# LoganWilliams1/mhm2_kmer_analysis_v2

Hardware: AMD Instinct MI355X
Metric: k-mers/sec (kcount stage) at k=21 (higher is better)
Workload: dtype u64

## Files before the change

### mhm2_kmer_analysis_v2_amd/csrc/kc_api.hip

```cpp
#include <hip/hip_runtime.h>

#include <math.h>
#include <stdio.h>
#include <stdlib.h>
#include <string.h>

#include <algorithm>
#include <new>
#include <thread>
#include <string>
#include <type_traits>
#include <unordered_map>
#include <vector>

#include "../../include/kcount_mi355.h"
#include "kc_bucketed.hpp"
#include "kc_shard.hpp"
#include "kc_wire6.hpp"
#include "kc_supermer.hpp"
#include "kc_ctg.hpp"
#include "kc_merge.hpp"
#include "kc_trim.hpp"
#include "kc_fastq.hpp"

// ... 30 lines not shown
                                               "kc_trim_sizes_kernel", "kc_merge_scan_kernel<trim>", "kc_trim_write_kernel"};
struct kt_pending {
  hipEvent_t start, stop;
  int kind;
};

struct kc_ctx {
  kc_config cfg;
  std::vector<kt_pending> kt_pend;
  uint64_t kt_launches[KT_COUNT];
  double kt_ms[KT_COUNT];
  int k, nl;
  int nl_ext;
  hipStream_t own_stream, stream;
  uint8_t *arena;
  size_t arena_bytes;
  uint64_t capacity;
  Table table;
  uint64_t *d_ctrs;
  uint64_t *h_ctrs;
  uint64_t *d_tile_first;
  uint64_t *d_out_plan;
  size_t tile_first_cap;
  uint8_t *d_stage_bases, *d_stage_quals;
  uint64_t *d_stage_offsets;
  size_t stage_bytes, stage_reads;
  struct {
    uint8_t *d_bases[2], *d_quals[2], *h_bases[2], *h_quals[2];
    uint64_t *d_offs[2], *h_offs[2];
    hipEvent_t copied[2], consumed[2], half[2];
    uint32_t lead_b[2], lead_q[2];
    bool used[2];
    hipStream_t copy_stream, copy_stream2;
    size_t cap_bytes, cap_reads;
    bool ready;
  } hp;
  uint64_t *d_out_keys;
  uint64_t *d_out_keys_ext;
  uint16_t *d_out_counts;
  uint8_t *d_out_left, *d_out_right;
  uint64_t out_cap, out_n;
  bool finalized;
  uint32_t *d_index;
  uint64_t index_cap;
  Table ctg_table;
  uint64_t ctg_cap;
// ... 376 lines not shown
  if (c->d_out_keys_ext) (void)hipFree(c->d_out_keys_ext);
  c->d_out_keys_ext = nullptr;
  if (c->d_out_counts) (void)hipFree(c->d_out_counts);
  if (c->d_out_left) (void)hipFree(c->d_out_left);
  if (c->d_out_right) (void)hipFree(c->d_out_right);
  c->d_out_keys = nullptr;
  c->d_out_counts = nullptr;
  c->d_out_left = c->d_out_right = nullptr;
  c->out_cap = c->out_n = 0;
}

extern "C" void kc_destroy(kc_ctx *c) {
  if (!c) return;
  (void)hipSetDevice(c->cfg.device);
  if (c->stream) (void)hipStreamSynchronize(c->stream);
  drain_kernel_times(c);
  free_results(c);
  if (c->arena) (void)hipFree(c->arena);
  if (c->d_ctrs) (void)hipFree(c->d_ctrs);
  if (c->d_w6cur) (void)hipFree(c->d_w6cur);
  if (c->d_l2snap) (void)hipFree(c->d_l2snap);
  if (c->h_ctrs) (void)hipHostFree(c->h_ctrs);
  if (c->d_tile_first) (void)hipFree(c->d_tile_first);
  if (c->d_out_plan) (void)hipFree(c->d_out_plan);
  if (c->d_stage_bases) (void)hipFree(c->d_stage_bases);
  if (c->d_stage_quals) (void)hipFree(c->d_stage_quals);
  if (c->d_stage_offsets) (void)hipFree(c->d_stage_offsets);
  if (c->d_synth) (void)hipFree(c->d_synth);
  if (c->d_sm_bytes) (void)hipFree(c->d_sm_bytes);
  if (c->d_sm_packed) (void)hipFree(c->d_sm_packed);
  if (c->d_sm_targets) (void)hipFree(c->d_sm_targets);
  if (c->d_sm_out) (void)hipFree(c->d_sm_out);
  if (c->d_sm_ctr) (void)hipFree(c->d_sm_ctr);
  if (c->d_mg) (void)hipFree(c->d_mg);
  if (c->d_ad) (void)hipFree(c->d_ad);
  if (c->d_tr) (void)hipFree(c->d_tr);
  if (c->d_fq_text) (void)hipFree(c->d_fq_text);
  if (c->d_fq_tiles) (void)hipFree(c->d_fq_tiles);
  if (c->d_fq_recs) (void)hipFree(c->d_fq_recs);
  host_pipe_free(c);
  free_ctg(c);
  bk_free(c, false);
  shard_free(c);
  if (c->d_cb) (void)hipFree(c->d_cb);
  if (c->h_cb) (void)hipHostFree(c->h_cb);
  if (c->own_stream) (void)hipStreamDestroy(c->own_stream);
// ... 307 lines not shown
    if (!rc) rc = bk_take(c, 10, (void **)&b.ovf2, b.ovf2_cap * w);
    if (!rc) rc = bk_take(c, 11, (void **)&b.done1, nseg * 4);
    if (!rc) rc = bk_take(c, 12, (void **)&b.used2, (size_t)g.P1 * 4);
    if (rc) return rc;
  }
  if (getenv("KC_DEBUG_ADDR"))
    fprintf(stderr, "kc arenas: rec1 %p (%zu MB) chain1 %p cnt1 %p rec2 %p chain2 %p ovf1 %p ovf2 %p\n", (void *)b.rec1, rec1_bytes >> 20,
            (void *)b.chain1, (void *)b.cnt1, (void *)b.rec2, (void *)b.chain2, (void *)b.ovf1, (void *)b.ovf2);
  c->bk_bytes = rec1_bytes + rec2_bytes + (b.ovf1_cap + b.ovf2_cap) * w + nseg * (g.L1MAX + 1) * 4 + (size_t)R * (g.L2MAX + 2) * 4;
  c->bk_capacity = bcap;
  c->bk_ready = true;
  c->bk_rot = 0;
  int rc = bk_empty_level1(c);
  if (!rc) rc = bk_empty_level2(c);
  return rc;
}

static int sync_cb(kc_ctx *c) {
  HIPCHK(hipMemcpyAsync(c->h_cb, c->d_cb, CB_COUNT * 8, hipMemcpyDeviceToHost, c->stream));
  HIPCHK(hipStreamSynchronize(c->stream));
  return KC_OK;
}

static int bk_ovf1_room(kc_ctx *c, uint64_t want, uint64_t *room) {
  if (c->ovf1_ub + want <= c->bb.ovf1_cap) {
    *room = c->bb.ovf1_cap - c->ovf1_ub;
    return KC_OK;
  }
  int rc = sync_cb(c);
  if (rc) return rc;
  if (c->h_cb[CB_FATAL] & ~(c->inc_on ? (uint64_t)FATAL_OVF2 : 0ULL)) {
    snprintf(g_last_error, sizeof(g_last_error), "k-mer buffer: records were lost (fatal bits %llu)", (unsigned long long)c->h_cb[CB_FATAL]);
    return KC_ERR_CAPACITY;
  }
  uint64_t used = std::min<uint64_t>(c->h_cb[CB_OVF1], c->bb.ovf1_cap);
  if (used && c->bb.ovf1_cap - used < want && !c->sh.extracting) {
    rc = ensure_room(c, used);
    if (rc) return rc;
    {
      KernelTimer kt(c, KT_FALLBACK);
      with_nl(c, [&](auto nl) {
        auto kern = with_cp<nl>(c, [&](auto cp) { return kc_ovf1_drain_kernel<nl, cp>; });
        hipLaunchKernelGGL(kern, dim3((unsigned)std::min<uint64_t>((used + TPB - 1) / TPB, 256 * 32)), dim3(TPB), 0, c->stream, c->gm, c->bb,
                           used, c->table, c->d_ctrs);
      });
    }
    HIPCHK(hipGetLastError());
    HIPCHK(hipMemsetAsync(c->d_cb + CB_OVF1, 0, 8, c->stream));
    used = 0;
  }
  c->ovf1_ub = used;
  *room = c->bb.ovf1_cap - used;
  return KC_OK;
}

template <typename K>
static int set_dyn_lds(K kernel, size_t bytes) {
  HIPCHK(hipFuncSetAttribute((const void *)kernel, hipFuncAttributeMaxDynamicSharedMemorySize, (int)bytes));
  return KC_OK;
}

template <int NL> static size_t lds_l1_reads() {
  return ((sizeof(L1LDS) + 15) & ~size_t(15)) + Rnd<NL>::STAGE_READS + ((size_t)WGB * Rnd<NL>::RPOS_READS + 64) * 2;
}
template <int NL> static size_t lds_bin_reads() { return (sizeof(L1LDS) + 15) & ~size_t(15); }
template <int NL> static size_t lds_l1_records() { return ((sizeof(L1RLDS) + 15) & ~size_t(15)) + Rnd<NL>::STAGE; }
template <int NL> static size_t lds_l2() { return ((sizeof(L2LDS) + 15) & ~size_t(15)) + Rnd<NL>::STAGE; }

template <int NL, int FMT>
static int launch_l1_reads_t(kc_ctx *c, const ExtractArgs &a, uint64_t nsuper) {
  const bool sh = c->cfg.rank_n > 1 && !c->sh.extracting;
  c->gm.own_lo = 0;
  c->gm.own_hi = PMAX;
  if (c->sh.extracting && c->cfg.rank_n > 1) {
    c->gm.own_lo = shard_first_bucket((uint32_t)c->cfg.rank_me, c->gm.P1, (uint32_t)c->cfg.rank_n);
    c->gm.own_hi = shard_first_bucket((uint32_t)c->cfg.rank_me + 1, c->gm.P1, (uint32_t)c->cfg.rank_n);
  }
  auto kern = with_cp<NL>(c, [&](auto cp) { return sh ? kc_l1_reads_kernel<NL, FMT, cp, true> : kc_l1_reads_kernel<NL, FMT, cp, false>; });
  const unsigned grid = (unsigned)std::min<uint64_t>(c->gm.G, nsuper);
  if constexpr (NL == 1) {
    if (c->gm.rec6) {
      auto kern16 = c->k == 21 ? (sh ? kc_l1_reads16_kernel<FMT, true, 21> : kc_l1_reads16_kernel<FMT, false, 21>)
                               : (sh ? kc_l1_reads16_kernel<FMT, true, 0> : kc_l1_reads16_kernel<FMT, false, 0>);
      int rc16 = set_dyn_lds(kern16, l1x16_lds_bytes());
      if (rc16) return rc16;
      KernelTimer kt(c, FMT == FMT_READS_UQ ? KT_L1_READS_UQ : KT_L1_READS16);
      hipLaunchKernelGGL(kern16, dim3(grid), dim3(WGB), l1x16_lds_bytes(), c->stream, a, c->gm, c->bb, nsuper, c->bk_rot, c->d_ctrs, c->d_cb);
      c->bk_rot = (uint32_t)((c->bk_rot + nsuper) % c->gm.G);
      return KC_OK;
    }
  }
  int rc = set_dyn_lds(kern, lds_l1_reads<NL>());
  if (rc) return rc;
  KernelTimer kt(c, FMT == FMT_READS_UQ ? KT_L1_READS_UQ : KT_L1_READS);
  hipLaunchKernelGGL(kern, dim3(grid), dim3(WGB), lds_l1_reads<NL>(), c->stream, a, c->gm, c->bb, nsuper, c->bk_rot, c->d_ctrs, c->d_cb);
  c->bk_rot = (uint32_t)((c->bk_rot + nsuper) % c->gm.G);
  return KC_OK;
}

static int launch_l1_reads(kc_ctx *c, const ExtractArgs &a, uint64_t ntiles, int fmt) {
  return with_fmt(fmt, [&](auto f) { return with_nl(c, [&](auto nl) { return launch_l1_reads_t<nl, f>(c, a, ntiles); }); });
}

template <int NL, int FMT>
static int launch_bin_reads_t(kc_ctx *c, const ExtractArgs &a, uint64_t nsuper) {
  auto kern = kc_bin_reads_kernel<NL, FMT>;
  int rc = set_dyn_lds(kern, lds_bin_reads<NL>());
  if (rc) return rc;
  const unsigned grid = (unsigned)std::min<uint64_t>((uint64_t)c->num_cus, nsuper);
  KernelTimer kt(c, KT_EXTRACT_BIN);
  hipLaunchKernelGGL(kern, dim3(grid), dim3(WGB), lds_bin_reads<NL>(), c->stream, a, nsuper, c->d_ctrs);
  return KC_OK;
}

static uint32_t bin_lg_pieces(const kc_ctx *c) { return c->wire6 ? wire6_lg_pieces((uint32_t)c->cfg.rank_n) : 0; }
static uint32_t bin_pieces(const kc_ctx *c) { return 1u << bin_lg_pieces(c); }

template <int FMT>
static int launch_bin16_t(kc_ctx *c, const ExtractArgs &a, uint64_t nsuper) {
  auto kern = c->k == 21 ? kc_bin16_kernel<FMT, 21> : kc_bin16_kernel<FMT, 0>;
  int rc = set_dyn_lds(kern, bin16_lds_bytes());
  if (rc) return rc;
  const unsigned grid = (unsigned)std::min<uint64_t>((uint64_t)c->num_cus, nsuper);
  KernelTimer kt(c, KT_BIN16);
// ... 507 lines not shown
        c->expect_host += *host_occ;
        total = c->expect_host;
      } else {
        rc = sync_ctrs(c);
        if (rc) return rc;
        if (c->h_ctrs[CTR_BAD_BASE]) return KC_ERR_BAD_BASE;
        total = c->h_ctrs[CTR_EXPECT];
        c->expect_host = total;
        c->expect_host_ok = true;
      }
      over_capacity = total - c->expect_base > c->bk_capacity;
      if (over_capacity && !c->sh.flow && c->expect_prev > c->expect_base && total - c->expect_prev <= c->bk_capacity) {
        rc = bk_make_room(c, c->expect_prev - c->expect_base);
        if (rc) return rc;
        c->expect_base = c->expect_prev;
        over_capacity = false;
      }
      c->expect_prev = total;
    } else {
      c->expect_host_ok = false;
    }
  }
  int64_t p0 = 0;
  while (p0 < end) {
    const bool bk = (mode == MODE_INSERT) && bk_active(c);
    const bool super = bk || mode == MODE_BIN;
    const uint64_t span = super ? (uint64_t)SUPER_SPAN : (uint64_t)TILE;
    uint64_t chunk_tiles;
    if (super) {
      chunk_tiles = (1ULL << 31) / span;
    } else {
      chunk_tiles = std::max<uint64_t>(64, (c->capacity / 4) / span);
      chunk_tiles = std::min<uint64_t>(chunk_tiles, (1ULL << 28) / span);
    }
    uint64_t nt = std::min<uint64_t>(chunk_tiles, ((uint64_t)(end - p0) + span - 1) / span);
    if (bk && over_capacity && c->sh.flow) {
      snprintf(g_last_error, sizeof(g_last_error), "shard flow: more k-mers than max_kmers_buffered (%llu): raise it, or use kc_extract_partition / kc_insert_records",
               (unsigned long long)c->bk_capacity);
      return KC_ERR_CAPACITY;
    }
    if (bk && over_capacity) {
      int rc = bk_drain_to_table(c);
      if (rc) return rc;
      continue;
    }
    if (bk) {
      uint64_t room = 0;
      int rc = bk_ovf1_room(c, nt * span, &room);
      if (rc) return rc;
      nt = std::max<uint64_t>(1, std::min<uint64_t>(nt, room / span));
      c->ovf1_ub += nt * span;
      if (room < span) {
        snprintf(g_last_error, sizeof(g_last_error), "overflow list smaller than one tile of %llu positions: raise ovf_capacity", (unsigned long long)span);
        return KC_ERR_CAPACITY;
      }
    }
    if (mode == MODE_INSERT && !bk) {
      int rc = ensure_room(c, nt * span);
      if (rc) return rc;
    }
    if (fmt != FMT_SEQBLOCK) {
      int rc = ensure_tile_first(c, nt);
      if (rc) return rc;
      {
        KernelTimer kt(c, KT_TILE_FIRST);
        hipLaunchKernelGGL(kc_tile_first_kernel, dim3((unsigned)((nt + 255) / 256)), dim3(256), 0, c->stream, d_offsets, nreads,
                           a.align, p0, (uint32_t)span, nt, c->d_tile_first);
      }
      a.tile_first = c->d_tile_first;
    }
    a.pos0 = p0;
    if (bk) {
      int rc = launch_l1_reads(c, a, nt, fmt);
      if (rc) return rc;
    } else if (mode == MODE_BIN) {
      int rc = launch_bin_reads(c, a, nt, fmt);
      if (rc) return rc;
    } else {
      launch_extract(c, a, (unsigned)nt, fmt);
    }
    HIPCHK(hipGetLastError());
    p0 += (int64_t)(nt * span);
    if (fmt != FMT_SEQBLOCK && p0 < end) HIPCHK(hipStreamSynchronize(c->stream));
  }
  return KC_OK;
}

static int raw_kmer_stats(kc_ctx *c, const uint64_t *d_offsets, uint64_t nreads, int mode) {
  if (!nreads) return KC_OK;
  unsigned nblk = (unsigned)std::min<uint64_t>((nreads + 255) / 256, 4096);
  hipLaunchKernelGGL(kc_read_stats_kernel, dim3(nblk), dim3(256), 0, c->stream, d_offsets, nreads, c->k, c->d_ctrs,
                     mode == MODE_INSERT ? 1u : 0u);
  c->num_gpu_calls++;
  HIPCHK(hipGetLastError());
  return KC_OK;
}

static int ensure_stage(kc_ctx *c, size_t bytes, size_t reads, bool need_quals) {
  if (bytes + 64 > c->stage_bytes) {
    if (c->d_stage_bases) HIPCHK(hipFree(c->d_stage_bases));
    if (c->d_stage_quals) HIPCHK(hipFree(c->d_stage_quals));
    c->d_stage_bases = c->d_stage_quals = nullptr;
    c->stage_bytes = 0;
    HIPCHK(hipMalloc((void **)&c->d_stage_bases, bytes + 64));
    HIPCHK(hipMalloc((void **)&c->d_stage_quals, bytes + 64));
    c->stage_bytes = bytes + 64;
// ... 2444 lines not shown
```

### mhm2_kmer_analysis_v2_amd/csrc/kc_bucketed.hpp

```cpp
#pragma once
#include "kc_kernels.hpp"

namespace kc {

constexpr int WGB = 1024;
constexpr int SUPER_SPAN = 16 * WGB - PRE - POST;
using TileSuper = TileGeo<WGB, SUPER_SPAN>;
static_assert(TileSuper::GPT == 1 && TileSuper::NGROUP == WGB, "one group per thread");
constexpr int PMAX = 1024;
constexpr int GMAX = 512;

template <int NL> struct Rnd {
  static constexpr int RPOS = NL == 1 ? 16 : NL == 2 ? 8 : 4;
  static constexpr int RPOS_READS = NL == 1 ? 8 : NL <= 3 ? 4 : 2;
  static constexpr size_t STAGE = ((size_t)WGB * RPOS + 64) * NL * 8;
  static constexpr size_t STAGE_READS = ((size_t)WGB * RPOS_READS + 64) * NL * 8;
};

struct Geom {
  uint32_t G, P1, P2, S;
  uint32_t log2CH1, log2CH2;
  uint32_t L1MAX, L2MAX;
  uint32_t A1;
  uint32_t A2;
// ... 10 lines not shown
  uint32_t *cnt1;
  uint32_t *used1;
  uint64_t *rec2;
  uint32_t *chain2;
  uint32_t *cnt2;
  uint32_t *base2;
  uint32_t *flag;
  uint64_t *ovf1;
  uint64_t *ovf2;
  uint64_t ovf1_cap, ovf2_cap;
  uint32_t *done1;
  uint32_t *used2;
};

constexpr uint32_t FLAT_MAX = 256;
struct FlatSrc {
  const uint32_t *cnt;
  const uint64_t *at;
  uint32_t F, nbo;
  uint32_t b_lo, b_hi;
};

enum {
  CB_OVF1 = 0, CB_OVF2, CB_FATAL, CB_FLAGGED_RECS, CB_DUMP, CB_ENTRIES, CB_OUT_RESERVED, CB_COUNT = 16
};
enum { FATAL_OVF1 = 1,
       FATAL_ARENA2 = 2,
       FATAL_OVF2 = 4 };


__device__ __forceinline__ uint32_t hash_b1(uint64_t h, const Geom &g) { return (((uint32_t)h & 0xFFFFu) * g.P1) >> 16; }
__device__ __forceinline__ uint32_t hash_b2(uint64_t h, const Geom &g) { return ((((uint32_t)h >> 16) & 0xFFFFu) * g.P2) >> 16; }
__device__ __forceinline__ uint32_t hash_slot(uint64_t h, uint32_t S) {
  return (uint32_t)(h >> 32) & (S - 1u);
}

__device__ __forceinline__ uint64_t cp_mix_rec(uint64_t keyrec, const Geom &g) {
  const uint32_t sh = 64u - g.k2;
  return (kc_feistel_fwd(keyrec >> sh, (int)(g.k2 >> 1)) << sh) | (keyrec & KC_EXT_MASK);
}
__device__ __forceinline__ uint64_t cp_unmix_rec(uint64_t mixrec, const Geom &g) {
  const uint32_t sh = 64u - g.k2;
  return (kc_feistel_inv(mixrec >> sh, (int)(g.k2 >> 1)) << sh) | (mixrec & KC_EXT_MASK);
}
__device__ __forceinline__ uint32_t cp_b1(uint64_t rec, const Geom &g) { return (uint32_t)(rec >> (64u - g.la)); }
__device__ __forceinline__ uint32_t cp_b2(uint64_t rec, const Geom &g) { return (uint32_t)(rec >> (64u - g.la - g.lb)) & (g.P2 - 1u); }
__device__ __forceinline__ uint32_t cp_pack32(uint64_t rec, const Geom &g) {
// ... 43 lines not shown
  const int tid = threadIdx.x;
  const int wave = __builtin_amdgcn_readfirstlane(tid >> 6);
  const uint32_t incl = wave_incl_scan(v);
  if (lane_id() == 63) S.wsum[wave] = incl;
  lds_barrier();
  const uint32_t w = (lane_id() < WGB / 64) ? S.wsum[lane_id()] : 0u;
  uint32_t wi = w;
  wi += (uint32_t)__builtin_amdgcn_update_dpp(0, (int)wi, 0x111, 0xF, 0xF, false);
  wi += (uint32_t)__builtin_amdgcn_update_dpp(0, (int)wi, 0x112, 0xF, 0xF, false);
  wi += (uint32_t)__builtin_amdgcn_update_dpp(0, (int)wi, 0x114, 0xF, 0xF, false);
  wi += (uint32_t)__builtin_amdgcn_update_dpp(0, (int)wi, 0x118, 0xF, 0xF, false);
  const uint32_t wave_pre = (uint32_t)__builtin_amdgcn_readlane((int)(wi - w), wave);
  const uint32_t total = (uint32_t)__builtin_amdgcn_readlane((int)wi, WGB / 64 - 1);
  if (tid == 0) S.total = total;
  return incl - v + wave_pre;
}

struct SplitLDS {
  uint32_t hist[2][PMAX + 64];
  uint4 dst[PMAX];
  uint32_t arena_used;
  uint32_t arena_top;
  ScanLDS scan;
};

__device__ __forceinline__ uint32_t hist_rank(SplitLDS &L, int buf, uint32_t b, bool valid) {
  return atomicAdd(&L.hist[buf][valid ? b : (uint32_t)PMAX + lane_id()], 1u);
}

#ifdef KC_STAMPS
#define KC_SPLIT_STAMP(k)                                                                 \
  if (threadIdx.x == 0 && D.stamps) {                                                     \
    const unsigned long long tn_ = __builtin_amdgcn_s_memtime();                          \
    atomicAdd((unsigned long long *)&D.stamps[k], tn_ - *D.tprev);                        \
    *D.tprev = tn_;                                                                       \
  }
#else
#define KC_SPLIT_STAMP(k)
#endif

struct ChainDest {
#ifdef KC_STAMPS
  uint64_t *stamps;
  unsigned long long *tprev;
#endif
  uint64_t *arena;
// ... 190 lines not shown
__device__ __forceinline__ ChainDest l1_dest(const Geom &gm, const BucketBufs &bb, uint32_t g) {
  ChainDest D;
#ifdef KC_STAMPS
  D.stamps = nullptr;
  D.tprev = nullptr;
#endif
  D.arena = bb.rec1 + (((size_t)g * gm.A1) << gm.log2CH1) * NL;
  D.chain = bb.chain1 + (size_t)g * gm.P1 * gm.L1MAX;
  D.log2CH = gm.log2CH1;
  D.LMAX = gm.L1MAX;
  D.arena_cap = gm.A1;
  D.arena_base = 0;
  D.own_lo = gm.own_lo;
  D.own_hi = gm.own_hi;
  return D;
}

__device__ __forceinline__ ChainDest l1_dest6(const Geom &gm, const BucketBufs &bb, uint32_t g) {
  ChainDest D = l1_dest<1>(gm, bb, g);
  D.arena = reinterpret_cast<uint64_t *>(reinterpret_cast<uint8_t *>(bb.rec1) + (((size_t)g * gm.A1) << gm.log2CH1) * 6);
  return D;
}

template <int NL, bool CP>
__device__ __forceinline__ void l1_overflow(const Geom &gm, const BucketBufs &bb, uint64_t *cb, const uint64_t (&r)[NL]) {
  const uint64_t o = atomicAdd((unsigned long long *)&cb[CB_OVF1], 1ULL);
  if (o < bb.ovf1_cap) {
#pragma unroll
    for (int w = 0; w < NL; w++) bb.ovf1[o * NL + w] = (CP && w == 0) ? cp_unmix_rec(r[w], gm) : r[w];
  } else {
    atomicOr((unsigned long long *)&cb[CB_FATAL], (unsigned long long)FATAL_OVF1);
  }
}

template <int KT, int RPOS, bool SH, class TL>
__device__ __forceinline__ void cp_run_fixed(const TL &L, int lp0, bool active, const Geom &gm, const ExtractArgs &a, uint32_t (&lo)[RPOS],
                                             uint32_t (&bk)[RPOS]) {
  const int K = KT ? KT : (int)a.k;
  const int NB = RPOS + K + 1;
  static_assert(RPOS + KT + 1 <= 32 && RPOS % 8 == 0 && PRE % 8 == 0, "the window must fit one word and never start word-aligned");
  const uint64_t *W = reinterpret_cast<const uint64_t *>(L.codes);
  const uint32_t *OK = reinterpret_cast<const uint32_t *>(L.ok);
  const int p = lp0 - 1, q = p >> 5, s = p & 31;
  const uint64_t w0 = W[q], w1 = W[q + 1];
  const uint32_t ok0 = OK[q], ok1 = OK[q + 1], g0 = L.gap[q], g1 = L.gap[q + 1];
  const uint64_t Wn = (w0 << (2 * s)) | (w1 >> (64 - 2 * s));
// ... 49 lines not shown
  constexpr uint64_t MID = ((1ULL << (2 * K)) - 1ULL) << 2;
  constexpr uint64_t CMP = (K & 1) ? (MID | 3ULL) : MID;
  uint32_t okm = 0;
#pragma unroll
  for (int j = 0; j < RPOS; j++) {
    const uint64_t x = Wn >> (64 - 2 * (j + K + 2)), y = Rn >> (64 - 2 * (RPOS - 1 - j + K + 2));
    const bool swap = (y & CMP) < (x & CMP);
    const uint64_t sel = swap ? y : x;
    const uint32_t na = (nok >> j) & 1u, nb = (nok >> (j + K + 1)) & 1u;
    const uint32_t le = ((uint32_t)(sel >> (2 * K + 2)) & 3u) | ((swap ? nb : na) << 2);
    const uint32_t re = ((uint32_t)sel & 3u) | ((swap ? na : nb) << 2);
    const uint64_t key = (sel >> 2) << (64 - 2 * K);
    const uint64_t kk[1] = {key};
    h[j] = kc_hash<1>(kk);
    rec[j] = key | (uint64_t)((le & 4u) ? 4u : le) | ((uint64_t)((re & 4u) ? 4u : re) << 3);
    const bool valid = active && ((gapw >> (j + 1)) & ((1u << (K + 1)) - 1u)) == 0u;
    okm |= valid ? (1u << j) : 0u;
  }
  return okm;
}

template <int NL, int FMT, bool CP, bool SH>
__global__ __launch_bounds__(WGB) void kc_l1_reads_kernel(ExtractArgs a, Geom gm, BucketBufs bb, uint64_t nsuper, uint32_t rot,
                                                          uint64_t *ctrs, uint64_t *cb) {
  extern __shared__ __align__(16) uint8_t smem[];
  L1LDS &L = *reinterpret_cast<L1LDS *>(smem);
  uint64_t *sorted = reinterpret_cast<uint64_t *>(smem + ((sizeof(L1LDS) + 15) & ~size_t(15)));
  uint16_t *sbucket = CP ? nullptr : reinterpret_cast<uint16_t *>(smem + ((sizeof(L1LDS) + 15) & ~size_t(15)) + Rnd<NL>::STAGE_READS);
  constexpr int RPOS = Rnd<NL>::RPOS_READS;
  const int tid = threadIdx.x;
  const uint32_t g = (blockIdx.x + rot) % gm.G, P1 = gm.P1;
  ChainDest D = l1_dest<NL>(gm, bb, g);
#ifdef KC_STAMPS
  unsigned long long tprev_ = __builtin_amdgcn_s_memtime();
  D.stamps = cb + 8;
  D.tprev = &tprev_;
#endif
  ChainState cst = split_load_state(L.sp, P1, bb.cnt1 + (size_t)g * P1, D.chain, D.LMAX, D.log2CH, bb.used1[g], bb.used1[gm.G + g]);
  __syncthreads();
  uint32_t n_ins = 0;
  int buf = 0;
  TileRaw<TileSuper> raw;
  auto first_of = [&](uint64_t st) -> uint64_t { return (FMT != FMT_SEQBLOCK && st < nsuper) ? a.tile_first[st] : 0; };
  tile_prefetch<FMT, TileSuper>(raw, a, a.pos0 + (int64_t)blockIdx.x * SUPER_SPAN, tid, first_of(blockIdx.x), blockIdx.x < nsuper);
  uint64_t next_first = first_of((uint64_t)blockIdx.x + gridDim.x);
  constexpr int RUNS = SUPER_SPAN / RPOS;
  static_assert(SUPER_SPAN % RPOS == 0, "runs must tile the span");
  constexpr int NROUND = (RUNS + WGB - 1) / WGB;
  for (int64_t it = -1;; it++) {
    const uint64_t st = (uint64_t)blockIdx.x + (uint64_t)(it < 0 ? 0 : it) * gridDim.x;
    const bool work = it >= 0;
    if (work && st >= nsuper) break;
#pragma unroll 1
    for (int round = 0; round < NROUND; round++) {
      uint64_t rec[RPOS][NL];
      uint32_t br[RPOS];
      uint32_t total = 0;
      if (work) {
      const int run_id = round * WGB + tid;
      const bool active = run_id < RUNS;
      const int lp0 = PRE + (active ? run_id : 0) * RPOS;
      KmerRun<NL> run;
      run_begin<NL>(run, L.tile, lp0, a.k);
#pragma unroll
      for (int j = 0; j < RPOS; j++) {
        uint64_t h = 0;
        uint32_t owner = 0;
        bool valid = run_kmer<NL, !CP>(run, j, lp0, a.k, rec[j], h, SH ? a.rank_n : 1u, SH ? a.reference_owner : 0u, SH ? &owner : nullptr) && active;
        if (SH) {
          if (CP && !a.reference_owner) {
            uint64_t key[NL];
#pragma unroll
            for (int w = 0; w < NL; w++) key[w] = rec[j][w];
            key[NL - 1] &= ~KC_EXT_MASK;
            owner = kc_owner_of_hash(kc_hash<NL>(key), a.rank_n);
          }
          valid = valid && owner == a.rank_me;
        }
        if (CP) rec[j][0] = cp_mix_rec(rec[j][0], gm);
        br[j] = valid ? (CP ? cp_b1(rec[j][0], gm) : hash_b1(h, gm)) : ~0u;
        if (j + 1 < RPOS) run_advance<NL>(run, j, lp0, a.k);
      }
#pragma unroll
      for (int j = 0; j < RPOS; j++) {
        const bool valid = br[j] != ~0u;
        const uint32_t rank = hist_rank(L.sp, buf, br[j] & (PMAX - 1), valid);
        br[j] = valid ? (br[j] | (rank << 10)) : ~0u;
        n_ins += valid ? 1u : 0u;
      }
      KC_SPLIT_STAMP(0)
      lds_barrier();
      total = split_stage<NL, RPOS>(
          L.sp, sorted, sbucket, buf, P1,
          [&](int j, uint64_t (&o)[NL]) {
#pragma unroll
            for (int w = 0; w < NL; w++) o[w] = rec[j][w];
          },
          br, D, cst);
      }
      if (round == NROUND - 1) {
        const uint64_t nst = work ? st + gridDim.x : st;
        tile_encode<FMT, TileSuper>(L.tile, raw, a, a.pos0 + (int64_t)nst * SUPER_SPAN, ctrs, tid, nst < nsuper);
        tile_prefetch<FMT, TileSuper>(raw, a, a.pos0 + (int64_t)(nst + gridDim.x) * SUPER_SPAN, tid, next_first, nst + gridDim.x < nsuper);
        next_first = first_of(nst + 2 * (uint64_t)gridDim.x);
        KC_SPLIT_STAMP(5)
      }
      if (work) {
        split_copy_out<NL>(
            L.sp, sorted, sbucket, total, D, [&](const uint64_t (&r)[NL]) { return cp_b1(r[0], gm); },
            [&](uint32_t, const uint64_t (&r)[NL]) { l1_overflow<NL, CP>(gm, bb, cb, r); },
            [&](size_t i, const uint64_t (&r)[NL]) { store_words<NL>(D.arena, i, r); });
        buf ^= 1;
      }
    }
  }
  if ((uint32_t)tid < P1) bb.cnt1[(size_t)g * P1 + tid] = cst.cur;
  if (tid == 0) {
    bb.used1[g] = min(L.sp.arena_used, gm.A1);
    bb.used1[gm.G + g] = min(L.sp.arena_top, gm.A1);
  }
  for (int o = 32; o > 0; o >>= 1) n_ins += __shfl_down(n_ins, o);
  if (lane_id() == 0 && n_ins) atomicAdd((unsigned long long *)&ctrs[CTR_INSERTED], (unsigned long long)n_ins);
}

constexpr int R16 = 16;
constexpr uint32_t ST16_MAIN = (uint32_t)WGB * R16 + PMAX;
constexpr uint32_t ST16_SLOTS = ST16_MAIN + 64;
static_assert(SUPER_SPAN % R16 == 0 && SUPER_SPAN / R16 <= WGB, "one run of sixteen positions per thread covers the super-tile");
static_assert(ST16_MAIN < 65536, "staging positions fit 16 bits");
constexpr size_t l1x16_lds_bytes() { return ((sizeof(L1LDS) + 15) & ~size_t(15)) + (size_t)ST16_SLOTS * 6; }

template <class MidFn>
__device__ __forceinline__ uint32_t split_stage_pairs(SplitLDS &L, uint32_t *slo, uint16_t *sbk, int buf, uint32_t P, const uint32_t (&lo)[R16],
                                                      const uint32_t (&br)[R16], const ChainDest &D, ChainState &st, MidFn mid) {
  const int tid = fresh_tid();
  KC_SPLIT_STAMP(1)
  const uint32_t v = ((uint32_t)tid < P) ? L.hist[buf][tid] : 0u;
  const uint32_t excl = block_excl_scan((v + 1u) & ~1u, L.scan);
  const uint32_t CHm = (1u << D.log2CH) - 1u;
  if ((uint32_t)tid < P) {
    const uint32_t base = st.cur;
    uint32_t fit = v;
    const uint64_t room = ((uint64_t)D.LMAX << D.log2CH) - base;
// ... 121 lines not shown
        const uint64_t bh = (uint64_t)(bk2[u] & (PMAX - 1)) << shb;
        const uint64_t ra = bh | ((uint64_t)l0 << shl) | (uint64_t)((bk2[u] >> 10) & 63u);
        const uint64_t rb = bh | ((uint64_t)l1 << shl) | (uint64_t)(bk2[u] >> 26);
        const bool f0 = j < fit, real1 = j + 1u < v, f1 = real1 && j + 1u < fit;
        if (!f0) overflow(ra);
        if (real1 && !(f0 && f1 && at1 == at0 + 1u)) {
          if (f1) {
            Rec6 r;
            r.lo = l1;
            r.bk = (uint16_t)(bk2[u] >> 16);
            *reinterpret_cast<Rec6 *>(arena0 + (size_t)at1 * 6) = r;
          } else {
            overflow(rb);
          }
        }
      }
    }
  }
  KC_SPLIT_STAMP(4)
}

template <int FMT, bool SH, int KK>
__global__ __launch_bounds__(WGB) void kc_l1_reads16_kernel(ExtractArgs a, Geom gm, BucketBufs bb, uint64_t nsuper, uint32_t rot, uint64_t *ctrs,
                                                            uint64_t *cb) {
  extern __shared__ __align__(16) uint8_t smem[];
  L1LDS &L = *reinterpret_cast<L1LDS *>(smem);
  uint32_t *slo = reinterpret_cast<uint32_t *>(smem + ((sizeof(L1LDS) + 15) & ~size_t(15)));
  uint16_t *sbk = reinterpret_cast<uint16_t *>(slo + ST16_SLOTS);
  const int tid = threadIdx.x;
  const uint32_t g = (blockIdx.x + rot) % gm.G, P1 = gm.P1;
  ChainDest D = l1_dest6(gm, bb, g);
#ifdef KC_STAMPS
  unsigned long long tprev_ = __builtin_amdgcn_s_memtime();
  D.stamps = cb + 8;
  D.tprev = &tprev_;
#endif
  ChainState cst = split_load_state(L.sp, P1, bb.cnt1 + (size_t)g * P1, D.chain, D.LMAX, D.log2CH, bb.used1[g], bb.used1[gm.G + g]);
  __syncthreads();
  uint32_t n_ins = 0;
  int buf = 0;
  TileRaw<TileSuper> raw;
  auto first_of = [&](uint64_t st) -> uint64_t { return (FMT != FMT_SEQBLOCK && st < nsuper) ? a.tile_first[st] : 0; };
  tile_prefetch<FMT, TileSuper>(raw, a, a.pos0 + (int64_t)blockIdx.x * SUPER_SPAN, tid, first_of(blockIdx.x), blockIdx.x < nsuper);
  uint64_t next_first = first_of((uint64_t)blockIdx.x + gridDim.x);
  constexpr int RUNS = SUPER_SPAN / R16;
  {
    const int ft = fresh_tid();
    tile_encode<FMT, TileSuper>(L.tile, raw, a, a.pos0 + (int64_t)blockIdx.x * SUPER_SPAN, ctrs, ft, blockIdx.x < nsuper);
    tile_prefetch<FMT, TileSuper>(raw, a, a.pos0 + (int64_t)((uint64_t)blockIdx.x + gridDim.x) * SUPER_SPAN, ft, next_first,
                                  (uint64_t)blockIdx.x + gridDim.x < nsuper);
    next_first = first_of((uint64_t)blockIdx.x + 2 * (uint64_t)gridDim.x);
  }
  for (uint64_t st = blockIdx.x; st < nsuper; st += gridDim.x) {
    uint32_t lo[R16], br[R16];
    const bool active = tid < RUNS;
    const int lp0 = PRE + (active ? tid : 0) * R16;
    {
      uint32_t l8[8], b8[8];
      cp_run_fixed<KK, 8, SH>(L.tile, lp0, active, gm, a, l8, b8);
#pragma unroll
      for (int j = 0; j < 8; j++) {
        lo[j] = l8[j];
        br[j] = b8[j];
      }
      cp_run_fixed<KK, 8, SH>(L.tile, lp0 + 8, active, gm, a, l8, b8);
#pragma unroll
      for (int j = 0; j < 8; j++) {
        lo[8 + j] = l8[j];
        br[8 + j] = b8[j];
      }
    }
#pragma unroll
    for (int j = 0; j < R16; j++) {
      const bool valid = br[j] != ~0u;
      const uint32_t rank = hist_rank(L.sp, buf, br[j] & (PMAX - 1), valid);
      br[j] = valid ? (br[j] | (rank << 16)) : ~0u;
      n_ins += valid ? 1u : 0u;
    }
    KC_SPLIT_STAMP(0)
    lds_barrier();
    const int ft = fresh_tid();
    const uint64_t nst = st + gridDim.x;
    tile_encode_clear<TileSuper>(L.tile, raw, ft);
    const uint32_t total = split_stage_pairs(L.sp, slo, sbk, buf, P1, lo, br, D, cst, [&]() {
      tile_encode_fill<FMT, TileSuper>(L.tile, raw, a, a.pos0 + (int64_t)nst * SUPER_SPAN, ctrs, ft, nst < nsuper);
      tile_prefetch<FMT, TileSuper>(raw, a, a.pos0 + (int64_t)(nst + gridDim.x) * SUPER_SPAN, ft, next_first, nst + gridDim.x < nsuper);
      next_first = first_of(nst + 2 * (uint64_t)gridDim.x);
    });
    split_copy_out_pairs(L.sp, slo, sbk, total, D, gm, [&](uint64_t r) {
      const uint64_t rr[1] = {r};
      l1_overflow<1, true>(gm, bb, cb, rr);
    });
    buf ^= 1;
  }
  if ((uint32_t)tid < P1) bb.cnt1[(size_t)g * P1 + tid] = cst.cur;
  if (tid == 0) {
    bb.used1[g] = min(L.sp.arena_used, gm.A1);
    bb.used1[gm.G + g] = min(L.sp.arena_top, gm.A1);
  }
  for (int o = 32; o > 0; o >>= 1) n_ins += __shfl_down(n_ins, o);
  if (lane_id() == 0 && n_ins) atomicAdd((unsigned long long *)&ctrs[CTR_INSERTED], (unsigned long long)n_ins);
}

template <int NL, int R>
__device__ __forceinline__ void split_round_flat(SplitLDS &L, int buf, uint32_t P, const uint64_t (&rec)[R][NL], const uint32_t (&br)[R],
                                                 uint64_t *records, uint64_t seg_cap, uint64_t *cursors, uint64_t *overflow_flag) {
  const int tid = threadIdx.x;
  if ((uint32_t)tid < P) {
    const uint32_t v = L.hist[buf][tid];
    uint64_t base = 0;
    if (v) base = atomicAdd((unsigned long long *)&cursors[tid], (unsigned long long)v);
    const uint64_t room = base < seg_cap ? seg_cap - base : 0;
    uint4 d;
    d.x = (uint32_t)base;
    d.y = (uint32_t)(base >> 32);
    d.z = (uint64_t)v <= room ? v : (uint32_t)room;
    d.w = 0;
    L.dst[tid] = d;
    L.hist[buf ^ 1][tid] = 0;
  }
  lds_barrier();
#pragma unroll
// ... 1537 lines not shown
```

Baseline: 99.07 billion.

## Let L1 insert kernel self-bound on overflow space instead of host chunking

Replaces host-side chunking of the bucketed L1 insert, which sized each launch by worst-case overflow room and synchronized between chunks. The kernel now polls the overflow counter and stops early when a threshold is reached, saving per-block resume positions. The host then drains the overflow and relaunches. The tile-first table is also computed once for the whole remaining range, which removes the per-chunk stream synchronize. The cost is an extra atomic poll per super-tile, a host sync after each launch, and more complex resume logic.

New measurement: 100.1 billion (median of 3 runs). No clear change (+1.0%).

```diff
diff --git a/mhm2_kmer_analysis_v2_amd/csrc/kc_api.hip b/mhm2_kmer_analysis_v2_amd/csrc/kc_api.hip
--- a/mhm2_kmer_analysis_v2_amd/csrc/kc_api.hip
+++ b/mhm2_kmer_analysis_v2_amd/csrc/kc_api.hip
@@ -76,6 +76,8 @@
   uint64_t *d_tile_first;
   uint64_t *d_out_plan;
   size_t tile_first_cap;
+  uint64_t *d_l1_next;
+  size_t l1_next_cap;
   uint8_t *d_stage_bases, *d_stage_quals;
   uint64_t *d_stage_offsets;
   size_t stage_bytes, stage_reads;
@@ -498,6 +500,7 @@
   if (c->d_l2snap) (void)hipFree(c->d_l2snap);
   if (c->h_ctrs) (void)hipHostFree(c->h_ctrs);
   if (c->d_tile_first) (void)hipFree(c->d_tile_first);
+  if (c->d_l1_next) (void)hipFree(c->d_l1_next);
   if (c->d_out_plan) (void)hipFree(c->d_out_plan);
   if (c->d_stage_bases) (void)hipFree(c->d_stage_bases);
   if (c->d_stage_quals) (void)hipFree(c->d_stage_quals);
@@ -851,6 +854,8 @@
   return KC_OK;
 }
 
+static int bk_ovf1_drain(kc_ctx *c, uint64_t used);
+
 static int bk_ovf1_room(kc_ctx *c, uint64_t want, uint64_t *room) {
   if (c->ovf1_ub + want <= c->bb.ovf1_cap) {
     *room = c->bb.ovf1_cap - c->ovf1_ub;
@@ -864,7 +869,18 @@
   }
   uint64_t used = std::min<uint64_t>(c->h_cb[CB_OVF1], c->bb.ovf1_cap);
   if (used && c->bb.ovf1_cap - used < want && !c->sh.extracting) {
-    rc = ensure_room(c, used);
+    rc = bk_ovf1_drain(c, used);
+    if (rc) return rc;
+    used = 0;
+  }
+  c->ovf1_ub = used;
+  *room = c->bb.ovf1_cap - used;
+  return KC_OK;
+}
+
+static int bk_ovf1_drain(kc_ctx *c, uint64_t used) {
+  if (used) {
+    int rc = ensure_room(c, used);
     if (rc) return rc;
     {
       KernelTimer kt(c, KT_FALLBACK);
@@ -876,10 +892,8 @@
     }
     HIPCHK(hipGetLastError());
     HIPCHK(hipMemsetAsync(c->d_cb + CB_OVF1, 0, 8, c->stream));
-    used = 0;
-  }
-  c->ovf1_ub = used;
-  *room = c->bb.ovf1_cap - used;
+  }
+  c->ovf1_ub = 0;
   return KC_OK;
 }
 
@@ -897,7 +911,7 @@
 template <int NL> static size_t lds_l2() { return ((sizeof(L2LDS) + 15) & ~size_t(15)) + Rnd<NL>::STAGE; }
 
 template <int NL, int FMT>
-static int launch_l1_reads_t(kc_ctx *c, const ExtractArgs &a, uint64_t nsuper) {
+static int launch_l1_reads_t(kc_ctx *c, const ExtractArgs &a, uint64_t nsuper, const L1Bound &lb) {
   const bool sh = c->cfg.rank_n > 1 && !c->sh.extracting;
   c->gm.own_lo = 0;
   c->gm.own_hi = PMAX;
@@ -914,21 +928,52 @@
       int rc16 = set_dyn_lds(kern16, l1x16_lds_bytes());
       if (rc16) return rc16;
       KernelTimer kt(c, FMT == FMT_READS_UQ ? KT_L1_READS_UQ : KT_L1_READS16);
-      hipLaunchKernelGGL(kern16, dim3(grid), dim3(WGB), l1x16_lds_bytes(), c->stream, a, c->gm, c->bb, nsuper, c->bk_rot, c->d_ctrs, c->d_cb);
-      c->bk_rot = (uint32_t)((c->bk_rot + nsuper) % c->gm.G);
+      hipLaunchKernelGGL(kern16, dim3(grid), dim3(WGB), l1x16_lds_bytes(), c->stream, a, c->gm, c->bb, nsuper, c->bk_rot, c->d_ctrs, c->d_cb, lb);
       return KC_OK;
     }
   }
   int rc = set_dyn_lds(kern, lds_l1_reads<NL>());
   if (rc) return rc;
   KernelTimer kt(c, FMT == FMT_READS_UQ ? KT_L1_READS_UQ : KT_L1_READS);
-  hipLaunchKernelGGL(kern, dim3(grid), dim3(WGB), lds_l1_reads<NL>(), c->stream, a, c->gm, c->bb, nsuper, c->bk_rot, c->d_ctrs, c->d_cb);
-  c->bk_rot = (uint32_t)((c->bk_rot + nsuper) % c->gm.G);
-  return KC_OK;
-}
-
-static int launch_l1_reads(kc_ctx *c, const ExtractArgs &a, uint64_t ntiles, int fmt) {
-  return with_fmt(fmt, [&](auto f) { return with_nl(c, [&](auto nl) { return launch_l1_reads_t<nl, f>(c, a, ntiles); }); });
+  hipLaunchKernelGGL(kern, dim3(grid), dim3(WGB), lds_l1_reads<NL>(), c->stream, a, c->gm, c->bb, nsuper, c->bk_rot, c->d_ctrs, c->d_cb, lb);
+  return KC_OK;
+}
+
+static int launch_l1_reads(kc_ctx *c, const ExtractArgs &a, uint64_t ntiles, int fmt, const L1Bound &lb) {
+  return with_fmt(fmt, [&](auto f) { return with_nl(c, [&](auto nl) { return launch_l1_reads_t<nl, f>(c, a, ntiles, lb); }); });
+}
+
+static int l1_reads_self_bounded(kc_ctx *c, const ExtractArgs &a, uint64_t nt, int fmt) {
+  const size_t G = c->gm.G;
+  if (G > c->l1_next_cap) {
+    if (c->d_l1_next) HIPCHK(hipFree(c->d_l1_next));
+    c->d_l1_next = nullptr;
+    c->l1_next_cap = 0;
+    HIPCHK(hipMalloc((void **)&c->d_l1_next, G * 8));
+    c->l1_next_cap = G;
+  }
+  L1Bound lb;
+  lb.next = c->d_l1_next;
+  lb.stop_at = c->bb.ovf1_cap - 2 * (uint64_t)G * SUPER_SPAN;
+  lb.resumed = 0;
+  for (;;) {
+    int rc = launch_l1_reads(c, a, nt, fmt, lb);
+    if (rc) return rc;
+    HIPCHK(hipGetLastError());
+    rc = sync_cb(c);
+    if (rc) return rc;
+    if (c->h_cb[CB_FATAL] & ~(c->inc_on ? (uint64_t)FATAL_OVF2 : 0ULL)) {
+      snprintf(g_last_error, sizeof(g_last_error), "k-mer buffer: records were lost (fatal bits %llu)", (unsigned long long)c->h_cb[CB_FATAL]);
+      return KC_ERR_CAPACITY;
+    }
+    const uint64_t used = std::min<uint64_t>(c->h_cb[CB_OVF1], c->bb.ovf1_cap);
+    c->ovf1_ub = used;
+    if (!c->h_cb[CB_L1_STOPPED]) return KC_OK;
+    rc = bk_ovf1_drain(c, used);
+    if (rc) return rc;
+    HIPCHK(hipMemsetAsync(c->d_cb + CB_L1_STOPPED, 0, 8, c->stream));
+    lb.resumed = 1;
+  }
 }
 
 template <int NL, int FMT>
@@ -1482,12 +1527,16 @@
     }
   }
   int64_t p0 = 0;
+  uint64_t tf_span = 0;
+  int64_t tf_p0 = 0;
   while (p0 < end) {
     const bool bk = (mode == MODE_INSERT) && bk_active(c);
     const bool super = bk || mode == MODE_BIN;
     const uint64_t span = super ? (uint64_t)SUPER_SPAN : (uint64_t)TILE;
     uint64_t chunk_tiles;
-    if (super) {
+    if (bk) {
+      chunk_tiles = ~0ULL;
+    } else if (super) {
       chunk_tiles = (1ULL << 31) / span;
     } else {
       chunk_tiles = std::max<uint64_t>(64, (c->capacity / 4) / span);
@@ -1504,7 +1553,8 @@
       if (rc) return rc;
       continue;
     }
-    if (bk) {
+    const bool self_bounded = bk && !c->sh.extracting && c->bb.ovf1_cap >= 4 * (uint64_t)c->gm.G * span && nt * span > c->bb.ovf1_cap;
+    if (bk && !self_bounded) {
       uint64_t room = 0;
       int rc = bk_ovf1_room(c, nt * span, &room);
       if (rc) return rc;
@@ -1520,19 +1570,28 @@
       if (rc) return rc;
     }
     if (fmt != FMT_SEQBLOCK) {
-      int rc = ensure_tile_first(c, nt);
-      if (rc) return rc;
-      {
-        KernelTimer kt(c, KT_TILE_FIRST);
-        hipLaunchKernelGGL(kc_tile_first_kernel, dim3((unsigned)((nt + 255) / 256)), dim3(256), 0, c->stream, d_offsets, nreads,
-                           a.align, p0, (uint32_t)span, nt, c->d_tile_first);
+      if (tf_span != span) {
+        if (tf_span) HIPCHK(hipStreamSynchronize(c->stream));
+        const uint64_t rest = ((uint64_t)(end - p0) + span - 1) / span;
+        int rc = ensure_tile_first(c, rest);
+        if (rc) return rc;
+        {
+          KernelTimer kt(c, KT_TILE_FIRST);
+          hipLaunchKernelGGL(kc_tile_first_kernel, dim3((unsigned)((rest + 255) / 256)), dim3(256), 0, c->stream, d_offsets, nreads,
+                             a.align, p0, (uint32_t)span, rest, c->d_tile_first);
+        }
+        tf_span = span;
+        tf_p0 = p0;
       }
-      a.tile_first = c->d_tile_first;
+      a.tile_first = c->d_tile_first + (uint64_t)(p0 - tf_p0) / span;
     }
     a.pos0 = p0;
     if (bk) {
-      int rc = launch_l1_reads(c, a, nt, fmt);
+      L1Bound host_bounded;
+      memset(&host_bounded, 0, sizeof(host_bounded));
+      int rc = self_bounded ? l1_reads_self_bounded(c, a, nt, fmt) : launch_l1_reads(c, a, nt, fmt, host_bounded);
       if (rc) return rc;
+      c->bk_rot = (uint32_t)((c->bk_rot + nt) % c->gm.G);
     } else if (mode == MODE_BIN) {
       int rc = launch_bin_reads(c, a, nt, fmt);
       if (rc) return rc;
@@ -1541,7 +1600,6 @@
     }
     HIPCHK(hipGetLastError());
     p0 += (int64_t)(nt * span);
-    if (fmt != FMT_SEQBLOCK && p0 < end) HIPCHK(hipStreamSynchronize(c->stream));
   }
   return KC_OK;
 }
diff --git a/mhm2_kmer_analysis_v2_amd/csrc/kc_bucketed.hpp b/mhm2_kmer_analysis_v2_amd/csrc/kc_bucketed.hpp
--- a/mhm2_kmer_analysis_v2_amd/csrc/kc_bucketed.hpp
+++ b/mhm2_kmer_analysis_v2_amd/csrc/kc_bucketed.hpp
@@ -56,7 +56,9 @@
 };
 
 enum {
-  CB_OVF1 = 0, CB_OVF2, CB_FATAL, CB_FLAGGED_RECS, CB_DUMP, CB_ENTRIES, CB_OUT_RESERVED, CB_COUNT = 16
+  CB_OVF1 = 0, CB_OVF2, CB_FATAL, CB_FLAGGED_RECS, CB_DUMP, CB_ENTRIES, CB_OUT_RESERVED,
+  CB_L1_STOPPED,
+  CB_COUNT = 16
 };
 enum { FATAL_OVF1 = 1,
        FATAL_ARENA2 = 2,
@@ -146,6 +148,7 @@
   uint32_t arena_used;
   uint32_t arena_top;
   ScanLDS scan;
+  uint32_t ovf_go;
 };
 
 __device__ __forceinline__ uint32_t hist_rank(SplitLDS &L, int buf, uint32_t b, bool valid) {
@@ -382,6 +385,24 @@
   return D;
 }
 
+struct L1Bound {
+  uint64_t *next;
+  uint64_t stop_at;
+  uint32_t resumed;
+};
+__device__ __forceinline__ uint64_t l1_ovf_used(uint64_t *cb) { return atomicOr((unsigned long long *)&cb[CB_OVF1], 0ULL); }
+__device__ __forceinline__ uint64_t l1_bound_begin(SplitLDS &L, const L1Bound &lb, uint64_t *cb) {
+  if (threadIdx.x == 0) L.ovf_go = (!lb.next || l1_ovf_used(cb) <= lb.stop_at) ? 1u : 0u;
+  return (lb.next && lb.resumed) ? lb.next[blockIdx.x] : (uint64_t)blockIdx.x;
+}
+__device__ __forceinline__ bool l1_bound_go(const SplitLDS &L) { return __builtin_amdgcn_readfirstlane((int)L.ovf_go) != 0; }
+__device__ __forceinline__ void l1_bound_end(const L1Bound &lb, uint64_t *cb, uint64_t st, uint64_t nsuper) {
+  if (threadIdx.x == 0 && lb.next) {
+    lb.next[blockIdx.x] = st;
+    if (st < nsuper) atomicAdd((unsigned long long *)&cb[CB_L1_STOPPED], 1ULL);
+  }
+}
+
 template <int NL, bool CP>
 __device__ __forceinline__ void l1_overflow(const Geom &gm, const BucketBufs &bb, uint64_t *cb, const uint64_t (&r)[NL]) {
   const uint64_t o = atomicAdd((unsigned long long *)&cb[CB_OVF1], 1ULL);
@@ -477,7 +498,7 @@
 
 template <int NL, int FMT, bool CP, bool SH>
 __global__ __launch_bounds__(WGB) void kc_l1_reads_kernel(ExtractArgs a, Geom gm, BucketBufs bb, uint64_t nsuper, uint32_t rot,
-                                                          uint64_t *ctrs, uint64_t *cb) {
+                                                          uint64_t *ctrs, uint64_t *cb, L1Bound lb) {
   extern __shared__ __align__(16) uint8_t smem[];
   L1LDS &L = *reinterpret_cast<L1LDS *>(smem);
   uint64_t *sorted = reinterpret_cast<uint64_t *>(smem + ((sizeof(L1LDS) + 15) & ~size_t(15)));
@@ -492,25 +513,29 @@
   D.tprev = &tprev_;
 #endif
   ChainState cst = split_load_state(L.sp, P1, bb.cnt1 + (size_t)g * P1, D.chain, D.LMAX, D.log2CH, bb.used1[g], bb.used1[gm.G + g]);
+  const uint64_t st0 = l1_bound_begin(L.sp, lb, cb);
   __syncthreads();
   uint32_t n_ins = 0;
   int buf = 0;
   TileRaw<TileSuper> raw;
   auto first_of = [&](uint64_t st) -> uint64_t { return (FMT != FMT_SEQBLOCK && st < nsuper) ? a.tile_first[st] : 0; };
-  tile_prefetch<FMT, TileSuper>(raw, a, a.pos0 + (int64_t)blockIdx.x * SUPER_SPAN, tid, first_of(blockIdx.x), blockIdx.x < nsuper);
-  uint64_t next_first = first_of((uint64_t)blockIdx.x + gridDim.x);
+  tile_prefetch<FMT, TileSuper>(raw, a, a.pos0 + (int64_t)st0 * SUPER_SPAN, tid, first_of(st0), st0 < nsuper);
+  uint64_t next_first = first_of(st0 + gridDim.x);
   constexpr int RUNS = SUPER_SPAN / RPOS;
   static_assert(SUPER_SPAN % RPOS == 0, "runs must tile the span");
   constexpr int NROUND = (RUNS + WGB - 1) / WGB;
+  uint64_t st = st0;
   for (int64_t it = -1;; it++) {
-    const uint64_t st = (uint64_t)blockIdx.x + (uint64_t)(it < 0 ? 0 : it) * gridDim.x;
+    st = st0 + (uint64_t)(it < 0 ? 0 : it) * gridDim.x;
     const bool work = it >= 0;
     if (work && st >= nsuper) break;
+    if (work && !l1_bound_go(L.sp)) break;
 #pragma unroll 1
     for (int round = 0; round < NROUND; round++) {
       uint64_t rec[RPOS][NL];
       uint32_t br[RPOS];
       uint32_t total = 0;
+      uint64_t ovf_used = 0;
       if (work) {
       const int run_id = round * WGB + tid;
       const bool active = run_id < RUNS;
@@ -545,6 +570,7 @@
       }
       KC_SPLIT_STAMP(0)
       lds_barrier();
+      if (lb.next && round == NROUND - 1 && tid == 0) ovf_used = l1_ovf_used(cb);
       total = split_stage<NL, RPOS>(
           L.sp, sorted, sbucket, buf, P1,
           [&](int j, uint64_t (&o)[NL]) {
@@ -555,6 +581,7 @@
       }
       if (round == NROUND - 1) {
         const uint64_t nst = work ? st + gridDim.x : st;
+        if (lb.next && work && tid == 0) L.sp.ovf_go = ovf_used <= lb.stop_at ? 1u : 0u;
         tile_encode<FMT, TileSuper>(L.tile, raw, a, a.pos0 + (int64_t)nst * SUPER_SPAN, ctrs, tid, nst < nsuper);
         tile_prefetch<FMT, TileSuper>(raw, a, a.pos0 + (int64_t)(nst + gridDim.x) * SUPER_SPAN, tid, next_first, nst + gridDim.x < nsuper);
         next_first = first_of(nst + 2 * (uint64_t)gridDim.x);
@@ -574,6 +601,7 @@
     bb.used1[g] = min(L.sp.arena_used, gm.A1);
     bb.used1[gm.G + g] = min(L.sp.arena_top, gm.A1);
   }
+  l1_bound_end(lb, cb, st, nsuper);
   for (int o = 32; o > 0; o >>= 1) n_ins += __shfl_down(n_ins, o);
   if (lane_id() == 0 && n_ins) atomicAdd((unsigned long long *)&ctrs[CTR_INSERTED], (unsigned long long)n_ins);
 }
@@ -741,7 +769,7 @@
 
 template <int FMT, bool SH, int KK>
 __global__ __launch_bounds__(WGB) void kc_l1_reads16_kernel(ExtractArgs a, Geom gm, BucketBufs bb, uint64_t nsuper, uint32_t rot, uint64_t *ctrs,
-                                                            uint64_t *cb) {
+                                                            uint64_t *cb, L1Bound lb) {
   extern __shared__ __align__(16) uint8_t smem[];
   L1LDS &L = *reinterpret_cast<L1LDS *>(smem);
   uint32_t *slo = reinterpret_cast<uint32_t *>(smem + ((sizeof(L1LDS) + 15) & ~size_t(15)));
@@ -755,22 +783,24 @@
   D.tprev = &tprev_;
 #endif
   ChainState cst = split_load_state(L.sp, P1, bb.cnt1 + (size_t)g * P1, D.chain, D.LMAX, D.log2CH, bb.used1[g], bb.used1[gm.G + g]);
+  const uint64_t st0 = l1_bound_begin(L.sp, lb, cb);
   __syncthreads();
   uint32_t n_ins = 0;
   int buf = 0;
   TileRaw<TileSuper> raw;
   auto first_of = [&](uint64_t st) -> uint64_t { return (FMT != FMT_SEQBLOCK && st < nsuper) ? a.tile_first[st] : 0; };
-  tile_prefetch<FMT, TileSuper>(raw, a, a.pos0 + (int64_t)blockIdx.x * SUPER_SPAN, tid, first_of(blockIdx.x), blockIdx.x < nsuper);
-  uint64_t next_first = first_of((uint64_t)blockIdx.x + gridDim.x);
+  tile_prefetch<FMT, TileSuper>(raw, a, a.pos0 + (int64_t)st0 * SUPER_SPAN, tid, first_of(st0), st0 < nsuper);
+  uint64_t next_first = first_of(st0 + gridDim.x);
   constexpr int RUNS = SUPER_SPAN / R16;
   {
     const int ft = fresh_tid();
-    tile_encode<FMT, TileSuper>(L.tile, raw, a, a.pos0 + (int64_t)blockIdx.x * SUPER_SPAN, ctrs, ft, blockIdx.x < nsuper);
-    tile_prefetch<FMT, TileSuper>(raw, a, a.pos0 + (int64_t)((uint64_t)blockIdx.x + gridDim.x) * SUPER_SPAN, ft, next_first,
-                                  (uint64_t)blockIdx.x + gridDim.x < nsuper);
-    next_first = first_of((uint64_t)blockIdx.x + 2 * (uint64_t)gridDim.x);
-  }
-  for (uint64_t st = blockIdx.x; st < nsuper; st += gridDim.x) {
+    tile_encode<FMT, TileSuper>(L.tile, raw, a, a.pos0 + (int64_t)st0 * SUPER_SPAN, ctrs, ft, st0 < nsuper);
+    tile_prefetch<FMT, TileSuper>(raw, a, a.pos0 + (int64_t)(st0 + gridDim.x) * SUPER_SPAN, ft, next_first, st0 + gridDim.x < nsuper);
+    next_first = first_of(st0 + 2 * (uint64_t)gridDim.x);
+  }
+  uint64_t st = st0;
+  for (; st < nsuper; st += gridDim.x) {
+    if (!l1_bound_go(L.sp)) break;
     uint32_t lo[R16], br[R16];
     const bool active = tid < RUNS;
     const int lp0 = PRE + (active ? tid : 0) * R16;
@@ -801,10 +831,13 @@
     const int ft = fresh_tid();
     const uint64_t nst = st + gridDim.x;
     tile_encode_clear<TileSuper>(L.tile, raw, ft);
+    uint64_t ovf_used = 0;
+    if (lb.next && ft == 0) ovf_used = l1_ovf_used(cb);
     const uint32_t total = split_stage_pairs(L.sp, slo, sbk, buf, P1, lo, br, D, cst, [&]() {
       tile_encode_fill<FMT, TileSuper>(L.tile, raw, a, a.pos0 + (int64_t)nst * SUPER_SPAN, ctrs, ft, nst < nsuper);
       tile_prefetch<FMT, TileSuper>(raw, a, a.pos0 + (int64_t)(nst + gridDim.x) * SUPER_SPAN, ft, next_first, nst + gridDim.x < nsuper);
       next_first = first_of(nst + 2 * (uint64_t)gridDim.x);
+      if (lb.next && ft == 0) L.sp.ovf_go = ovf_used <= lb.stop_at ? 1u : 0u;
     });
     split_copy_out_pairs(L.sp, slo, sbk, total, D, gm, [&](uint64_t r) {
       const uint64_t rr[1] = {r};
@@ -817,6 +850,7 @@
     bb.used1[g] = min(L.sp.arena_used, gm.A1);
     bb.used1[gm.G + g] = min(L.sp.arena_top, gm.A1);
   }
+  l1_bound_end(lb, cb, st, nsuper);
   for (int o = 32; o > 0; o >>= 1) n_ins += __shfl_down(n_ins, o);
   if (lane_id() == 0 && n_ins) atomicAdd((unsigned long long *)&ctrs[CTR_INSERTED], (unsigned long long)n_ins);
 }
```
